# CSB5/XNA_Basecaller

Hardware: AMD Instinct MI355X
Metric: raw signal samples/sec basecalled, chunksize 10k (higher is better)
Workload: dtype f32 (feed-forward projections split-f16x3 MFMA, recurrent projections f16 MFMA + FP8 block-scaled correction MFMA, f32 accumulate; CRF decode f32)

## Files before the change

### xna_basecaller_amd/csrc/xb_encoder.hip

```cpp
#include "xb_enc_common.h"

namespace {

constexpr int CF_TT = 32;

__global__ __launch_bounds__(256) void conv_front_kernel(xb::ConvFrontParams p)
{
    extern __shared__ __attribute__((aligned(16))) unsigned char smem_raw[];
    const int tid = threadIdx.x;
    const int n = blockIdx.y;
    const int t0 = blockIdx.x * CF_TT;
    const int W = p.winlen, ST = p.stride, pad = W / 2, L = p.L;
    const int nq = (CF_TT - 1) * ST + W;
    const int q0 = t0 * ST - pad;
    float *sig = reinterpret_cast<float *>(smem_raw);
    float *a1 = sig + nq + 8;
    float *a2 = a1 + 4 * (nq + 4);
    float *w2s = a2 + 16 * nq;
    float *b2s = w2s + 320, *w1s = b2s + 16, *b1s = w1s + 20;

    for (int i = tid; i < 320; i += 256) w2s[i] = p.w2[i];
    if (tid < 16) b2s[tid] = p.b2[tid];
    if (tid < 20) w1s[tid] = p.w1[tid];
    if (tid < 4) b1s[tid] = p.b1[tid];
    const float *x = (p.signal2 && n >= p.split) ? p.signal2 + (size_t)(n - p.split) * L : p.signal + (size_t)n * L;
    for (int i = tid; i < nq + 8; i += 256) {
        const int pos = q0 - 4 + i;
        sig[i] = (pos >= 0 && pos < L) ? x[pos] : 0.0f;
    }
    __syncthreads();
    for (int i = tid; i < 4 * (nq + 4); i += 256) {
        const int c = i / (nq + 4), r = i % (nq + 4);
        const int pos = q0 - 2 + r;
        float v = 0.0f;
        if (pos >= 0 && pos < L) {
            float acc = b1s[c];
#pragma unroll
            for (int k = 0; k < 5; ++k) acc += w1s[c * 5 + k] * sig[r + k];
            v = silu(acc);
        }
        a1[c * (nq + 4) + r] = v;
    }
    __syncthreads();
    for (int i = tid; i < 16 * nq; i += 256) {
        const int c = i / nq, r = i % nq;
        const int pos = q0 + r;
        float v = 0.0f;
        if (pos >= 0 && pos < L) {
            float acc = b2s[c];
#pragma unroll
            for (int ci = 0; ci < 4; ++ci)
#pragma unroll
                for (int k = 0; k < 5; ++k) acc += w2s[(c * 4 + ci) * 5 + k] * a1[ci * (nq + 4) + r + k];
            v = silu(acc);
        }
        a2[c * nq + r] = v;
    }
    __syncthreads();
    const int kp = p.kp, kv = 16 * W, kq = kp / 4;
    for (int i = tid; i < CF_TT * kq; i += 256) {
        const int tt = i / kq, col = (i % kq) * 4;
        const int t = t0 + tt;
        if (t >= p.T) break;
        float v[4];
#pragma unroll
        for (int j = 0; j < 4; ++j) {
            const int cj = col + j;
            v[j] = cj < kv ? a2[(cj / W) * nq + tt * ST + cj % W] : 0.0f;
        }
        const size_t orow = (size_t)t * p.N + n;
        half_t hi[4];
        unsigned short hb[4];
        if (p.q8) {
            float lo[4];
#pragma unroll
            for (int j = 0; j < 4; ++j) {
                hi[j] = (half_t)v[j];
                lo[j] = clamp448((v[j] - (float)hi[j]) * 2048.0f);
                hb[j] = __builtin_bit_cast(unsigned short, hi[j]);
            }
            unsigned h8 = fp8_pair<false>(clamp448((float)hi[0]), clamp448((float)hi[1]), 0u);
            h8 = fp8_pair<true>(clamp448((float)hi[2]), clamp448((float)hi[3]), h8);
            unsigned l8 = fp8_pair<false>(lo[0], lo[1], 0u);
            l8 = fp8_pair<true>(lo[2], lo[3], l8);
            unsigned char *q = reinterpret_cast<unsigned char *>(p.a_lo) + q8_offset(orow, kp, col);
            *reinterpret_cast<unsigned *>(q) = h8;
            *reinterpret_cast<unsigned *>(q + 32) = l8;
        } else {
            unsigned short lb[4];
#pragma unroll
            for (int j = 0; j < 4; ++j) {
                half_t lo;
                split_f16(v[j], hi[j], lo);
                hb[j] = __builtin_bit_cast(unsigned short, hi[j]);
                lb[j] = __builtin_bit_cast(unsigned short, lo);
            }
            *reinterpret_cast<uint2 *>(p.a_lo + orow * kp + col) =
                make_uint2(lb[0] | ((unsigned)lb[1] << 16), lb[2] | ((unsigned)lb[3] << 16));
        }
        *reinterpret_cast<uint2 *>(p.a_hi + orow * kp + col) =
            make_uint2(hb[0] | ((unsigned)hb[1] << 16), hb[2] | ((unsigned)hb[3] << 16));
    }
}

constexpr int GBM = 256, GBN = 256, GBK = 32, GTHREADS = 512;


__host__ __device__ inline int gemm_super_n(int NT) { return NT % 2 == 0 ? 2 : (NT % 3 == 0 ? 3 : 1); }

__device__ __forceinline__ bool gemm_tile_origin(const xb::GemmParams &p, int &m0, int &n0)
{
    const int MT = (p.M + GBM - 1) / GBM, NT = (p.Nn + GBN - 1) / GBN;
    const int SN = gemm_super_n(NT), SM = 32 / SN;
    const int ngroups = (NT + SN - 1) / SN, msup = (MT + SM - 1) / SM;
    const int b = blockIdx.x, xcd = b & 7, j = b >> 3;
    const int q = (j >> 5) * 8 + xcd, w = j & 31;
    if (q >= msup * ngroups || w >= SM * SN) return false;
    const int mt = (q / ngroups) * SM + w / SN, nt = (q % ngroups) * SN + w % SN;
    if (mt >= MT || nt >= NT) return false;
    m0 = mt * GBM;
    n0 = nt * GBN;
    return true;
}

template <bool L16>
__device__ __forceinline__ constexpr int acc_row(int r) { return L16 ? (r & 7) + 16 * (r >> 3) : (r & 3) + 8 * (r >> 2); }

__device__ __forceinline__ void acc16_lines(const f32x4 (&a)[8][4], floatx16 (&o)[4][2])
{
    asm volatile("s_nop 7\n\ts_nop 7");
#pragma unroll
    for (int i = 0; i < 4; ++i)
#pragma unroll
        for (int jp = 0; jp < 2; ++jp)
#pragma unroll
            for (int ib = 0; ib < 2; ++ib)
#pragma unroll
                for (int r = 0; r < 4; ++r) {
                    float u = a[2 * i + ib][2 * jp][r], v = a[2 * i + ib][2 * jp + 1][r];
                    asm volatile("v_permlane16_swap_b32 %0, %1" : "+v"(u), "+v"(v));
                    o[i][jp][ib * 8 + r] = u;
                    o[i][jp][ib * 8 + 4 + r] = v;
                }
}

template <int EPI, bool L16 = false>
__device__ __forceinline__ void gemm_epilogue(const xb::GemmParams &p, const floatx16 (&acc)[4][2], int mw, int nw, int lane)
{
    constexpr int HS = L16 ? 8 : 4;
    if (mw >= p.M || nw >= p.Nn) return;
    float bj[2];
#pragma unroll
    for (int j = 0; j < 2; ++j) {
        const int n = nw + j * 32 + (lane & 31);
        bj[j] = (p.bias && n < p.Nn) ? p.bias[n] : 0.0f;
    }
    const bool interior = mw + 128 <= p.M && nw + 64 <= p.Nn;
    const bool out_q8 = p.out_fmt ? p.out_fmt == 2 : p.nsplit == 2;
    if (EPI == xb::EPI_BIAS_F32 && interior && (p.gin_n == 0 || p.gin_n >= 43)) {
        const int ld = p.gin_n ? 128 : p.ldc;
        float *tile;
        int c0 = 0, n = 1 << 30;
        long long wrap = 0;
        if (p.gin_n) {
            n = p.gin_n;
            const int t0 = mw / n;
            c0 = mw - t0 * n;
            const int MB = p.Nn >> 7;
            tile = p.out_f32 + (((size_t)t0 * MB + (size_t)(nw >> 7)) * n + c0) * 128 + (nw & 127);
            wrap = (long long)(MB - 1) * n * 128;
        } else {
            tile = p.out_f32 + (size_t)mw * p.ldc + nw;
        }
        const int loff = (HS * (lane >> 5)) * ld + (lane & 31);
        if (c0 + 128 <= n) {
#pragma unroll
            for (int i = 0; i < 4; ++i)
#pragma unroll
                for (int r = 0; r < 16; ++r) {
                    float *rowp = tile + (size_t)(i * 32 + acc_row<L16>(r)) * ld;
#pragma unroll
                    for (int j = 0; j < 2; ++j) __builtin_nontemporal_store(acc[i][j][r] + bj[j], rowp + loff + j * 32);
                }
        } else {
            const int cl = c0 + HS * (lane >> 5);
#pragma unroll
            for (int i = 0; i < 4; ++i)
#pragma unroll
                for (int r = 0; r < 16; ++r) {
                    const int rr = i * 32 + acc_row<L16>(r);
                    const int c = cl + rr;
                    const int k = (c >= n) + (c >= 2 * n) + (c >= 3 * n);
                    float *rowp = tile + (size_t)rr * ld + (long long)k * wrap;
#pragma unroll
                    for (int j = 0; j < 2; ++j) __builtin_nontemporal_store(acc[i][j][r] + bj[j], rowp + loff + j * 32);
                }
        }
        return;
    }
    if (EPI == xb::EPI_TANH_SCALE && interior && !p.expand) {
        float *tile = p.out_f32 + (size_t)mw * p.ldc + nw;
        const int loff = (HS * (lane >> 5)) * p.ldc + (lane & 31);
#pragma unroll
        for (int i = 0; i < 4; ++i)
#pragma unroll
            for (int r = 0; r < 16; ++r) {
                float *rowp = tile + (size_t)(i * 32 + acc_row<L16>(r)) * p.ldc;
#pragma unroll
                for (int j = 0; j < 2; ++j) rowp[loff + j * 32] = p.scale * fast_tanh(acc[i][j][r] + bj[j]);
            }
        return;
    }
    if (EPI == xb::EPI_SILU_SPLIT && interior) {
        const size_t tile = (size_t)mw * p.ldc + nw;
        const int loff = (HS * (lane >> 5)) * p.ldc + (lane & 31);
        unsigned char *q8base = reinterpret_cast<unsigned char *>(p.out_lo) + tile * 2;
        const int qoff = (HS * (lane >> 5)) * p.ldc * 2 + (lane & 31);
#pragma unroll
        for (int i = 0; i < 4; ++i)
#pragma unroll
            for (int r = 0; r < 16; ++r) {
                const size_t ro = (size_t)(i * 32 + acc_row<L16>(r)) * p.ldc;
#pragma unroll
                for (int j = 0; j < 2; ++j) {
                    const float v = silu(acc[i][j][r] + bj[j]);
                    if (out_q8) {
                        half_t hi;
                        unsigned char h8, l8;
                        q8_bytes(v, p.out_exp, hi, h8, l8);
                        p.out_hi[tile + ro + loff + j * 32] = hi;
                        unsigned char *q = q8base + ro * 2 + qoff + j * 64;
                        q[0] = h8;
                        q[32] = l8;
                    } else {
                        half_t hi, lo;
                        split_f16(v, hi, lo);
                        p.out_hi[tile + ro + loff + j * 32] = hi;
                        p.out_lo[tile + ro + loff + j * 32] = lo;
                    }
                }
            }
        return;
    }
#pragma unroll
    for (int i = 0; i < 4; ++i)
#pragma unroll
        for (int j = 0; j < 2; ++j) {
            const int n = nw + j * 32 + (lane & 31);
            if (n >= p.Nn) continue;
            const float bias = bj[j];
            int ocol = n;
            if (EPI == xb::EPI_TANH_SCALE && p.expand) ocol = (n / p.nb) * (p.nb + 1) + 1 + n % p.nb;
#pragma unroll
            for (int r = 0; r < 16; ++r) {
                const int m = mw + i * 32 + acc_row<L16>(r) + HS * (lane >> 5);
                if (m >= p.M) continue;
                const float v = acc[i][j][r] + bias;
                if (EPI == xb::EPI_BIAS_F32) {
                    p.out_f32[p.gin_n ? xb::gin_offset((size_t)m, n, p.gin_n, p.Nn) : (size_t)m * p.ldc + n] = v;
                } else if (EPI == xb::EPI_SILU_SPLIT) {
                    if (out_q8) {
                        half_t hi;
                        unsigned char h8, l8;
                        q8_bytes(silu(v), p.out_exp, hi, h8, l8);
                        unsigned char *q = reinterpret_cast<unsigned char *>(p.out_lo) + q8_offset((size_t)m, p.ldc, n);
                        p.out_hi[(size_t)m * p.ldc + n] = hi;
                        q[0] = h8;
                        q[32] = l8;
                    } else {
                        half_t hi, lo;
                        split_f16(silu(v), hi, lo);
                        p.out_hi[(size_t)m * p.ldc + n] = hi;
                        p.out_lo[(size_t)m * p.ldc + n] = lo;
                    }
                } else {
                    p.out_f32[(size_t)m * p.ldc + ocol] = p.scale * fast_tanh(v);
                    if (p.expand && n % p.nb == 0) p.out_f32[(size_t)m * p.ldc + ocol - 1] = p.blank;
                }
            }
        }
}

#define G8_BARRIER()                                   \
    do {                                               \
        __builtin_amdgcn_sched_barrier(0);             \
        __builtin_amdgcn_s_barrier();                  \
        __builtin_amdgcn_sched_barrier(0);             \
    } while (0)

template <int EPI, int NSPLIT>
__global__ __launch_bounds__(GTHREADS) void gemm8r_kernel(xb::GemmParams p)
{
    constexpr int NP = NSPLIT == 1 ? 1 : 2;
    constexpr int PARTB = 128 * 64;
    constexpr int HTB = NP * PARTB;
    extern __shared__ __attribute__((aligned(16))) unsigned char smem_raw[];
    const int tid = threadIdx.x, lane = tid & 63;
    const int wid = __builtin_amdgcn_readfirstlane(tid >> 6);
    const int wr = wid >> 2, wc = wid & 3;
    int m0, n0;
    if (!gemm_tile_origin(p, m0, n0)) return;
    const int nk = p.K / GBK;

    unsigned offs[4];
    {
        const int drow = 16 * wid + (lane >> 2), dch = ((lane & 3) ^ ((lane >> 4) & 3)) * 8;
        const int Mrem = p.M - 1 - m0, Nrem = p.Nn - 1 - n0;
        int r;
        r = drow;        offs[0] = (unsigned)(((r > Mrem ? Mrem : r) * p.lda + dch) * 2);
        r = 128 + drow;  offs[1] = (unsigned)(((r > Mrem ? Mrem : r) * p.lda + dch) * 2);
        r = drow;        offs[2] = (unsigned)(((r > Nrem ? Nrem : r) * p.ldb + dch) * 2);
        r = 128 + drow;  offs[3] = (unsigned)(((r > Nrem ? Nrem : r) * p.ldb + dch) * 2);
    }
    const unsigned char *const tA_hi = reinterpret_cast<const unsigned char *>(p.a_hi + (size_t)m0 * p.lda);
    const unsigned char *const tA_lo = reinterpret_cast<const unsigned char *>(p.a_lo + (size_t)m0 * p.lda);
    const unsigned char *const tB_hi = reinterpret_cast<const unsigned char *>(p.b_hi + (size_t)n0 * p.ldb);
    const unsigned char *const tB_lo = reinterpret_cast<const unsigned char *>(p.b_lo + (size_t)n0 * p.ldb);
    unsigned char *const wdst = smem_raw + wid * 1024;
    u32x4 st[4][NP];
    unsigned char *const ldst = wdst + lane * 16;
#define G8_LOAD(h, t)                                                                           \
    do {                                                                                        \
        const size_t kb_ = (size_t)(t) * (GBK * 2);                                             \
        st[(h)][0] = *reinterpret_cast<const u32x4 *>(((h) < 2 ? tA_hi : tB_hi) + kb_ + offs[(h)]); \
        if (NP == 2) st[(h)][1] = *reinterpret_cast<const u32x4 *>(((h) < 2 ? tA_lo : tB_lo) + kb_ + offs[(h)]); \
    } while (0)
#define G8_WRITE(h, t)                                                                          \
    do {                                                                                        \
        unsigned char *dst_ = ldst + (((h) * 2 + ((t) & 1)) * HTB);                             \
        *reinterpret_cast<u32x4 *>(dst_) = st[(h)][0];                                          \
        if (NP == 2) *reinterpret_cast<u32x4 *>(dst_ + PARTB) = st[(h)][1];                     \
    } while (0)

    unsigned la[2];
#pragma unroll
    for (int ks = 0; ks < 2; ++ks)
        la[ks] = (unsigned)((lane & 31) * 64 + (((2 * ks + (lane >> 5)) ^ ((lane >> 2) & 3)) * 16));
    constexpr bool S16 = NSPLIT == 3;
    const unsigned la16 = (unsigned)((lane & 15) * 64 + (((lane >> 4) ^ ((lane >> 2) & 3)) * 16));
    const unsigned char *const fragA = smem_raw + wr * 2 * HTB;
    const unsigned char *const fragB = smem_raw + (2 + (wc >> 1)) * 2 * HTB + (wc & 1) * 4096;

    unsigned lqa[2], lqb[2];
#pragma unroll
    for (int j = 0; j < 2; ++j) {
        const int h = lane >> 5, sw = (lane >> 2) & 3;
        lqa[j] = (unsigned)((lane & 31) * 64 + (((2 * h + j) ^ sw) * 16));
        lqb[j] = (unsigned)((lane & 31) * 64 + (((2 * (1 - h) + j) ^ sw) * 16));
    }
    const int sca = 127 - p.a_exp - 11, scb = 127 - p.b_exp;

    half8 ah[2][2], al[2][2], bh[2], bl[2];
    v8i aq[2], bq;
#define G8_READ_A(d, mh)                                                                                  \
    _Pragma("unroll") for (int i2 = 0; i2 < 2; ++i2) {                                                    \
        const unsigned char *t_ = fragA + (d) * HTB + ((mh) * 2 + i2) * 2048;                         \
        _Pragma("unroll") for (int ks = 0; ks < 2; ++ks) {                                                \
            ah[i2][ks] = *reinterpret_cast<const half8 *>(t_ + (S16 ? ks * 1024 + la16 : la[ks]));        \
            if (S16) al[i2][ks] = *reinterpret_cast<const half8 *>(t_ + PARTB + ks * 1024 + la16);       \
        }                                                                                                 \
        if (NSPLIT == 2) {                                                                                \
            const v4i x_ = *reinterpret_cast<const v4i *>(t_ + PARTB + lqa[0]);                           \
            const v4i y_ = *reinterpret_cast<const v4i *>(t_ + PARTB + lqa[1]);                           \
            aq[i2] = __builtin_shufflevector(x_, y_, 0, 1, 2, 3, 4, 5, 6, 7);                             \
        }                                                                                                 \
    }
#define G8_READ_B(d, n)                                                                                   \
    do {                                                                                                  \
        const unsigned char *t_ = fragB + (d) * HTB + (n) * 2048;                                     \
        _Pragma("unroll") for (int ks = 0; ks < 2; ++ks) {                                                \
            bh[ks] = *reinterpret_cast<const half8 *>(t_ + (S16 ? ks * 1024 + la16 : la[ks]));            \
            if (S16) bl[ks] = *reinterpret_cast<const half8 *>(t_ + PARTB + ks * 1024 + la16);           \
        }                                                                                                 \
        if (NSPLIT == 2) {                                                                                \
            const v4i x_ = *reinterpret_cast<const v4i *>(t_ + PARTB + lqb[0]);                           \
            const v4i y_ = *reinterpret_cast<const v4i *>(t_ + PARTB + lqb[1]);                           \
            bq = __builtin_shufflevector(x_, y_, 0, 1, 2, 3, 4, 5, 6, 7);                            \
        }                                                                                                 \
    } while (0)
#define G8_F16(i2, ks, n, A_, B_)                                                                         \
    acc[(mh_) * 2 + (i2)][(n)] = __builtin_amdgcn_mfma_f32_32x32x16_f16(A_[(i2)][(ks)], B_[(ks)], acc[(mh_) * 2 + (i2)][(n)], 0, 0, 0)
#define G8_S16(A_, B_, n)                                                                                 \
    _Pragma("unroll") for (int i4 = 0; i4 < 4; ++i4)                                                      \
        _Pragma("unroll") for (int j2 = 0; j2 < 2; ++j2)                                                  \
            acc16[mh_ * 4 + i4][(n) * 2 + j2] = __builtin_amdgcn_mfma_f32_16x16x32_f16(A_[i4 >> 1][i4 & 1], B_[j2], acc16[mh_ * 4 + i4][(n) * 2 + j2], 0, 0, 0)
#define G8_MFMA(mh, n)                                                                                    \
    do {                                                                                                  \
        constexpr int mh_ = (mh);                                                                         \
        __builtin_amdgcn_s_setprio(1);                                                                    \
        if constexpr (S16) {                                                                              \
            G8_S16(al, bh, n);                                                                            \
            G8_S16(ah, bl, n);                                                                            \
            G8_S16(ah, bh, n);                                                                            \
        } else if (NSPLIT == 2) {                                                                                \
            G8_F16(0, 0, n, ah, bh);                                                                      \
            G8_F16(1, 0, n, ah, bh);                                                                      \
            _Pragma("unroll") for (int i2 = 0; i2 < 2; ++i2) acc[mh_ * 2 + i2][(n)] =                     \
                __builtin_amdgcn_mfma_scale_f32_32x32x64_f8f6f4(aq[i2], bq, acc[mh_ * 2 + i2][(n)], 0, 0, 0, sca, 0, scb); \
            G8_F16(0, 1, n, ah, bh);                                                                      \
            G8_F16(1, 1, n, ah, bh);                                                                      \
        } else {                                                                                          \
            _Pragma("unroll") for (int ks = 0; ks < 2; ++ks) {                                            \
                G8_F16(0, ks, n, ah, bh);                                                                 \
                G8_F16(1, ks, n, ah, bh);                                                                 \
            }                                                                                             \
        }                                                                                                 \
        __builtin_amdgcn_s_setprio(0);                                                                    \
    } while (0)

    floatx16 acc[4][2];
    f32x4 acc16[8][4];
#pragma unroll
    for (int i = 0; i < 4; ++i)
#pragma unroll
        for (int j = 0; j < 2; ++j)
#pragma unroll
            for (int r = 0; r < 16; ++r) acc[i][j][r] = 0.0f;
#pragma unroll
    for (int i = 0; i < 8; ++i)
#pragma unroll
        for (int j = 0; j < 4; ++j)
#pragma unroll
            for (int r = 0; r < 4; ++r) acc16[i][j][r] = 0.0f;

#pragma unroll
    for (int h = 0; h < 4; ++h) G8_LOAD(h, 0);
#pragma unroll
    for (int h = 0; h < 4; ++h) G8_WRITE(h, 0);
#pragma unroll
    for (int h = 0; h < 4; ++h) G8_LOAD(h, nk > 1 ? 1 : 0);
    asm volatile("s_waitcnt lgkmcnt(0)" ::: "memory");
    G8_BARRIER();
    if (wr == 1) G8_BARRIER();
// ... 193 lines not shown
    _Pragma("unroll") for (int i_ = 0; i_ < 2; ++i_)                                            \
        _Pragma("unroll") for (int j_ = 0; j_ < 2; ++j_)                                        \
            _Pragma("unroll") for (int c_ = 0; c_ < 2; ++c_)                                    \
                acc16[(q) * 2 + i_][2 * j_ + c_] = __builtin_amdgcn_mfma_f32_16x16x32_f16(      \
                    A_[i_], __builtin_bit_cast(half8, bS[j_][(pc0) + c_]), acc16[(q) * 2 + i_][2 * j_ + c_], 0, 0, 0)
#define G4P_S16(AH_, AL_, q, bS)                                                                \
    do {                                                                                        \
        G4P_M16(AL_, q, bS, 0);                                                                 \
        G4P_M16(AH_, q, bS, 2);                                                                 \
        G4P_M16(AH_, q, bS, 0);                                                                 \
    } while (0)
#define G4P_WAIT8(n, bS)                                                                        \
    asm volatile("s_waitcnt vmcnt(%8)" : "+v"(bS[0][0]), "+v"(bS[1][0]), "+v"(bS[0][1]), "+v"(bS[1][1]), \
                 "+v"(bS[0][2]), "+v"(bS[1][2]), "+v"(bS[0][3]), "+v"(bS[1][3]) : "i"(n))
#define G4P_MFMA_BEGIN() do { G4P_SB(); __builtin_amdgcn_s_setprio(1); } while (0)
#define G4P_MFMA_END() do { __builtin_amdgcn_s_setprio(0); G4P_SB(); } while (0)

#define G4P_TILE(bS, t)                                                                         \
    do {                                                                                        \
        const unsigned char *const sa = smem_raw + cur * STB;                                   \
        const int t2_ = (t) + 2 < nk ? (t) + 2 : nk - 1;                                        \
        const unsigned char *const b2 = tB + (size_t)t2_ * bks;                                 \
         \
        const bool live_ = (t) + 2 < nk;                                                        \
        const unsigned vb_ = live_ ? voff0 : 0u;                                                \
        if ((t) == 0) G4P_STAMP(0);                                                             \
        if constexpr (!S16) {                                                                   \
            asm volatile("s_waitcnt vmcnt(%0)" ::"i"(2 * NB + NA) : "memory");                  \
            G4P_SB();                                                                           \
            __builtin_amdgcn_s_barrier();                                                       \
            G4P_SB();                                                                           \
            G4P_STAMP(1);                                                                       \
        }                                                                                       \
        if constexpr (NSPLIT == 2) {                                                            \
            dma_a(t2_, nxt2, live_);           \
             \
             \
            half8 h0[2], h1[2], g0[2], g1[2];                                                   \
            v8i q0[2], q1[2];                                                                   \
            G4P_RD_H(h0, sa, 0, 0, 0);                                                          \
            G4P_RD_H(h1, sa, 0, 1, 0);                                                          \
            G4P_WAIT2(INFL - 2, bS[0][0], bS[1][0]);                                            \
            G4P_MFMA_BEGIN();                                                                   \
            G4P_F16(h0, 0, bS, 0);                                                              \
            G4P_MFMA_END();                                                                     \
            G4P_RD_Q(q0, sa, 0);                                                                \
            G4P_RD_Q(q1, sa, 1);                                                                \
            G4P_MFMA_BEGIN();                                                                   \
            G4P_F16(h1, 1, bS, 0);                                                              \
            G4P_MFMA_END();                                                                     \
            G4P_LDB_GROUP_V(bS, vb_, b2, 0);                                                           \
            G4P_WAIT4(INFL - 4, bS[0][2], bS[0][3], bS[1][2], bS[1][3]);                        \
            G4P_MFMA_BEGIN();                                                                   \
            G4P_F8(q0, 0, bS);                                                                  \
            G4P_MFMA_END();                                                                     \
            G4P_RD_H(g0, sa, 0, 0, 1);                                                          \
            G4P_RD_H(g1, sa, 0, 1, 1);                                                          \
            G4P_MFMA_BEGIN();                                                                   \
            G4P_F8(q1, 1, bS);                                                                  \
            G4P_MFMA_END();                                                                     \
            G4P_LDB_GROUP_V(bS, vb_, b2, 2);                                                           \
            G4P_LDB_GROUP_V(bS, vb_, b2, 3);                                                           \
            G4P_WAIT2(INFL - 2, bS[0][1], bS[1][1]);                                            \
            G4P_MFMA_BEGIN();                                                                   \
            G4P_F16(g0, 0, bS, 1);                                                              \
            G4P_F16(g1, 1, bS, 1);                                                              \
            G4P_MFMA_END();                                                                     \
            G4P_LDB_GROUP_V(bS, vb_, b2, 1);                                                           \
        } else if constexpr (S16) {                                                             \
             \
             \
             \
             \
             \
             \
             \
             \
            half8 yh[2], yl[2];                                                                 \
            G4P_RD16(yl, sa, 1, 1);                                                             \
            G4P_RD16(yh, sa, 0, 1);                                                             \
            G4P_WAIT8(INFL - 8 - NA, bS);                                                       \
            G4P_STAMP(2);                                                                       \
            G4P_MFMA_BEGIN();                                                                   \
            G4P_S16(xh, xl, 0, bS);                                                             \
            G4P_MFMA_END();                                                                     \
            dma_a(t2_, nxt2, live_);                                                            \
            G4P_RD16(xl, sa, 1, 2);                                                             \
            G4P_RD16(xh, sa, 0, 2);                                                             \
            G4P_MFMA_BEGIN();                                                                   \
            G4P_S16(yh, yl, 1, bS);                                                             \
            G4P_MFMA_END();                                                                     \
            G4P_RD16(yl, sa, 1, 3);                                                             \
            G4P_RD16(yh, sa, 0, 3);                                                             \
            G4P_MFMA_BEGIN();                                                                   \
            G4P_S16(xh, xl, 2, bS);                                                             \
            G4P_MFMA_END();                                                                     \
            G4P_STAMP(3);                                                                       \
            asm volatile("s_waitcnt vmcnt(%0)\n\ts_waitcnt lgkmcnt(0)" ::"i"(NB + NA) : "memory"); \
            G4P_SB();                                                                           \
            __builtin_amdgcn_s_barrier();                                                       \
            G4P_SB();                                                                           \
            G4P_STAMP(1);                                                                       \
            const unsigned char *const sn = smem_raw + nxt1 * STB;                              \
            G4P_RD16(xl, sn, 1, 0);                                                             \
            G4P_RD16(xh, sn, 0, 0);                                                             \
            G4P_MFMA_BEGIN();                                                                   \
            G4P_M16(yl, 3, bS, 0);                                                              \
            G4P_M16(yh, 3, bS, 2);                                                              \
            G4P_MFMA_END();                                                                     \
            G4P_LDB_GROUP_V(bS, vb_, b2, 2);                                                    \
            G4P_LDB_GROUP_V(bS, vb_, b2, 3);                                                    \
            G4P_MFMA_BEGIN();                                                                   \
            G4P_M16(yh, 3, bS, 0);                                                              \
            G4P_MFMA_END();                                                                     \
            G4P_LDB_GROUP_V(bS, vb_, b2, 0);                                                    \
            G4P_LDB_GROUP_V(bS, vb_, b2, 1);                                                    \
        } else {                                                                                \
             \
             \
             \
             \
            half8 ah0[2], ah1[2];                                                               \
            G4P_RD_H(ah0, sa, 0, 0, 0);                                                         \
            G4P_RD_H(ah1, sa, 0, 1, 0);                                                         \
            _Pragma("unroll") for (int ks = 0; ks < 2; ++ks) {                                  \
                 \
                 \
                constexpr int LA_ = NA;                                                         \
                if (ks == 0) G4P_WAIT2(INFL - 2 - LA_, bS[0][0], bS[1][0]);                     \
                else G4P_WAIT2(INFL - 2, bS[0][1], bS[1][1]);                                   \
                G4P_MFMA_BEGIN();                                                               \
                G4P_F16(ah0, 0, bS, ks);                                                        \
                G4P_MFMA_END();                                                                 \
                if (ks == 0) {                                                                  \
                    dma_a(t2_, nxt2, live_);                                                    \
                    G4P_RD_H(ah0, sa, 0, 0, 1);                                                 \
                }                                                                               \
                G4P_MFMA_BEGIN();                                                               \
                G4P_F16(ah1, 1, bS, ks);                                                        \
                G4P_MFMA_END();                                                                 \
                if (ks == 0) {                                                                  \
                    G4P_RD_H(ah1, sa, 0, 1, 1);                                                 \
                    G4P_LDB_GROUP_V(bS, vb_, b2, 0);                                            \
                } else {                                                                        \
                    G4P_LDB_GROUP_V(bS, vb_, b2, 1);                                            \
                }                                                                               \
            }                                                                                   \
        }                                                                                       \
        if constexpr (!S16) asm volatile("s_waitcnt lgkmcnt(0)" ::: "memory");                  \
        G4P_STAMP(3);                                                                           \
        { const int c_ = cur; cur = nxt1; nxt1 = nxt2; nxt2 = c_; }                             \
    } while (0)

    if (__builtin_amdgcn_readfirstlane(n0 + wid * 64 >= p.Nn ? 1 : 0)) {
        dma_a(0, 0);
        dma_a(nk > 1 ? 1 : 0, 1);
        int c0 = 0, c1 = 1, c2 = 2;
#pragma unroll 1
        for (int t = 0; t < nk + (S16 ? 1 : 0); ++t) {
            asm volatile("s_waitcnt vmcnt(%0)" ::"i"(NA) : "memory");
            __builtin_amdgcn_s_barrier();
            dma_a(t + 2 < nk ? t + 2 : nk - 1, c2, t + 2 < nk);
            const int c_ = c0; c0 = c1; c1 = c2; c2 = c_;
        }
        asm volatile("s_waitcnt vmcnt(0)" ::: "memory");
        return;
    }

    int cur = 0, nxt1 = 1, nxt2 = 2;
    {
        const int t1 = nk > 1 ? 1 : 0;
        const unsigned char *const b0 = tB, *const b1 = tB + (size_t)t1 * bks;
        dma_a(0, 0);
        if constexpr (NSPLIT == 2) {
            G4P_LDB_GROUP(bE, b0, 0); G4P_LDB_GROUP(bE, b0, 2); G4P_LDB_GROUP(bE, b0, 3); G4P_LDB_GROUP(bE, b0, 1);
        } else if constexpr (S16) {
            G4P_LDB_GROUP(bE, b0, 2); G4P_LDB_GROUP(bE, b0, 3); G4P_LDB_GROUP(bE, b0, 0); G4P_LDB_GROUP(bE, b0, 1);
        } else {
            G4P_LDB_GROUP(bE, b0, 0); G4P_LDB_GROUP(bE, b0, 1);
        }
        dma_a(t1, 1);
        if constexpr (NSPLIT == 2) {
            G4P_LDB_GROUP(bO, b1, 0); G4P_LDB_GROUP(bO, b1, 2); G4P_LDB_GROUP(bO, b1, 3); G4P_LDB_GROUP(bO, b1, 1);
        } else if constexpr (S16) {
            G4P_LDB_GROUP(bO, b1, 2); G4P_LDB_GROUP(bO, b1, 3); G4P_LDB_GROUP(bO, b1, 0); G4P_LDB_GROUP(bO, b1, 1);
        } else {
            G4P_LDB_GROUP(bO, b1, 0); G4P_LDB_GROUP(bO, b1, 1);
        }
    }
    if constexpr (S16) {
        asm volatile("s_waitcnt vmcnt(%0)" ::"i"(2 * NB + NA) : "memory");
        G4P_SB();
        __builtin_amdgcn_s_barrier();
        G4P_SB();
        G4P_RD16(xl, smem_raw, 1, 0);
        G4P_RD16(xh, smem_raw, 0, 0);
    }
    int t = 0;
#pragma unroll 1
    for (; t + 1 < nk; t += 2) {
        G4P_TILE(bE, t);
        G4P_TILE(bO, t + 1);
    }
    if (t < nk) G4P_TILE(bE, t);
    if constexpr (NSPLIT == 1)
        asm volatile("s_waitcnt vmcnt(0)" : "+v"(bE[0][0]), "+v"(bE[1][0]), "+v"(bE[0][1]), "+v"(bE[1][1]),
                       "+v"(bO[0][0]), "+v"(bO[1][0]), "+v"(bO[0][1]), "+v"(bO[1][1]) :: "memory");
    else
        asm volatile("s_waitcnt vmcnt(0)" : "+v"(bE[0][0]), "+v"(bE[1][0]), "+v"(bE[0][1]), "+v"(bE[1][1]),
                       "+v"(bE[0][2]), "+v"(bE[1][2]), "+v"(bE[0][3]), "+v"(bE[1][3]),
                       "+v"(bO[0][0]), "+v"(bO[1][0]), "+v"(bO[0][1]), "+v"(bO[1][1]),
                       "+v"(bO[0][2]), "+v"(bO[1][2]), "+v"(bO[0][3]), "+v"(bO[1][3]) :: "memory");
    G4P_SB();
#undef G4P_TILE
#undef G4P_LDB
#undef G4P_LDB_GROUP
#undef G4P_LDB_GROUP_V
#undef G4P_WAIT2
#undef G4P_WAIT4
#undef G4P_RD_H
#undef G4P_RD16
#undef G4P_M16
#undef G4P_S16
#undef G4P_WAIT8
#undef G4P_RD_Q
#undef G4P_F16
#undef G4P_F8
#undef G4P_MFMA_BEGIN
#undef G4P_MFMA_END
#undef G4P_SB

    int lane_e = lane, mw_e = m0, nw_e = n0 + wid * 64;
    asm volatile("" : "+v"(lane_e), "+s"(mw_e), "+s"(nw_e));
    if constexpr (S16) acc16_lines(acc16, acc);
    gemm_epilogue<EPI, S16>(p, acc, mw_e, nw_e, lane_e);
#ifdef XB_GEMM_STAMPS
    if (NSPLIT == 3) {
        asm volatile("s_waitcnt vmcnt(0)" ::: "memory");
        G4P_STAMP(4);
        if (tid == 0) {
            for (int i = 0; i < 5; ++i) atomicAdd(&g_gemm_stamps[i], st_acc[i]);
            atomicAdd(&g_gemm_stamps[5], (unsigned long long)(__builtin_amdgcn_s_getreg(4 | (0 << 6) | (3 << 11)) & 1u));
            atomicAdd(&g_gemm_stamps[6], 1ull);
            atomicAdd(&g_gemm_stamps[7], (unsigned long long)nk);
        }
    }
#endif
}

template <int EPI, int NSPLIT>
hipError_t launch_gemm_ns(const xb::GemmParams &p, hipStream_t stream)
{
    const int MT = (p.M + GBM - 1) / GBM, NT = (p.Nn + GBN - 1) / GBN;
    const int SN = gemm_super_n(NT), SM = 32 / SN;
    const int supers = ((NT + SN - 1) / SN) * ((MT + SM - 1) / SM);
    dim3 grid(8 * 32 * ((supers + 7) / 8)), block(GTHREADS);
    const size_t lds = (size_t)2 * 4 * (NSPLIT == 1 ? 1 : 2) * 128 * 64;
    (void)hipFuncSetAttribute(reinterpret_cast<const void *>(&gemm8r_kernel<EPI, NSPLIT>),
                              hipFuncAttributeMaxDynamicSharedMemorySize, (int)lds);
    hipLaunchKernelGGL((gemm8r_kernel<EPI, NSPLIT>), grid, block, lds, stream, p);
    return hipGetLastError();
}

template <int EPI, int NSPLIT>
hipError_t launch_gemm4p_ns(const xb::GemmParams &p, hipStream_t stream)
{
    const int MT = (p.M + G4_BM - 1) / G4_BM, NT = (p.Nn + G4_BN - 1) / G4_BN;
    const int snw = p.sn > 0 ? p.sn : gemm_super_n(NT);
    const int SN = NT < snw ? NT : snw, SM = 64 / SN;
    const int supers = ((NT + SN - 1) / SN) * ((MT + SM - 1) / SM);
    dim3 grid(8 * 64 * ((supers + 7) / 8)), block(G4_THREADS);
    size_t lds = (size_t)3 * (NSPLIT == 1 ? 1 : 2) * 128 * 64;
    if (p.one_per_cu) {
        lds = 96 * 1024;
        (void)hipFuncSetAttribute(reinterpret_cast<const void *>(&gemm4p_kernel<EPI, NSPLIT>),
                                  hipFuncAttributeMaxDynamicSharedMemorySize, (int)lds);
    }
    hipLaunchKernelGGL((gemm4p_kernel<EPI, NSPLIT>), grid, block, lds, stream, p);
    return hipGetLastError();
}

template <int EPI>
hipError_t launch_gemm_epi(const xb::GemmParams &p, hipStream_t stream)
{
    if (p.b4) {
        switch (p.nsplit) {
        case 1: return launch_gemm4p_ns<EPI, 1>(p, stream);
        case 2: return launch_gemm4p_ns<EPI, 2>(p, stream);
        default: return launch_gemm4p_ns<EPI, 3>(p, stream);
        }
    }
    switch (p.nsplit) {
    case 1: return launch_gemm_ns<EPI, 1>(p, stream);
    case 2: return launch_gemm_ns<EPI, 2>(p, stream);
    default: return launch_gemm_ns<EPI, 3>(p, stream);
    }
}

}


namespace xb {

#ifdef XB_GEMM_STAMPS
void gemm_read_stamps(unsigned long long out[8], bool reset)
{
    hipMemcpyFromSymbol(out, HIP_SYMBOL(g_gemm_stamps), sizeof(unsigned long long) * 8);
    if (reset) {
        unsigned long long z[8] = {};
        hipMemcpyToSymbol(HIP_SYMBOL(g_gemm_stamps), z, sizeof z);
    }
}
#endif

hipError_t launch_conv_front(const ConvFrontParams &p, hipStream_t stream)
{
    if (p.N < 1 || p.T < 1 || p.kp < 16 * p.winlen || p.kp % 32 != 0) return hipErrorInvalidValue;
    const int nq = (CF_TT - 1) * p.stride + p.winlen;
    const size_t lds = sizeof(float) * ((size_t)(nq + 8) + 4 * (nq + 4) + 16 * (size_t)nq + 360);
    if (lds > 60000) return hipErrorInvalidValue;
    dim3 grid((p.T + CF_TT - 1) / CF_TT, p.N), block(256);
    hipLaunchKernelGGL(conv_front_kernel, grid, block, lds, stream, p);
    return hipGetLastError();
}

hipError_t launch_gemm(const GemmParams &p, int epilogue, hipStream_t stream)
{
    if (p.M < 1 || p.Nn < 1 || p.K < GBK || p.K % GBK != 0 || p.lda % 8 != 0 || p.ldb % 8 != 0 ||
        p.lda < p.K || p.ldb < p.K)
        return hipErrorInvalidValue;
    if (p.nsplit < 1 || p.nsplit > 3) return hipErrorInvalidValue;
    switch (epilogue) {
    case EPI_BIAS_F32: return launch_gemm_epi<EPI_BIAS_F32>(p, stream);
    case EPI_SILU_SPLIT: return launch_gemm_epi<EPI_SILU_SPLIT>(p, stream);
    case EPI_TANH_SCALE: return launch_gemm_epi<EPI_TANH_SCALE>(p, stream);
    default: return hipErrorInvalidValue;
    }
}

}
```

Baseline: 43.28 million.

## Overlap GEMM epilogue stores with final k-tile MFMAs in split-f16 path

Refactors the GEMM epilogue into a struct with per-row-block store methods. The S16 kernel path peels the last k-tile and interleaves its MFMA groups with accumulator permutation and stores for completed row blocks, so epilogue global writes overlap the tail compute. It also reorders the B prefetch for odd tile counts and removes redundant DMA and extra barrier iterations in the idle-wave path. This adds register pressure and complexity in the tail and risks hazards around the permlane swaps on accumulators that are still being written.

Result: no change. 43.68 million, median of 6 (+0.9%).

```diff
diff --git a/xna_basecaller_amd/csrc/xb_encoder.hip b/xna_basecaller_amd/csrc/xb_encoder.hip
--- a/xna_basecaller_amd/csrc/xb_encoder.hip
+++ b/xna_basecaller_amd/csrc/xb_encoder.hip
@@ -126,66 +126,97 @@
 template <bool L16>
 __device__ __forceinline__ constexpr int acc_row(int r) { return L16 ? (r & 7) + 16 * (r >> 3) : (r & 3) + 8 * (r >> 2); }
 
+__device__ __forceinline__ void acc16_block(const f32x4 (&a)[8][4], floatx16 (&o)[2], int i)
+{
+    asm volatile("s_nop 7\n\ts_nop 7\n\ts_nop 7");
+#pragma unroll
+    for (int jp = 0; jp < 2; ++jp)
+#pragma unroll
+        for (int ib = 0; ib < 2; ++ib)
+#pragma unroll
+            for (int r = 0; r < 4; ++r) {
+                float u = a[2 * i + ib][2 * jp][r], v = a[2 * i + ib][2 * jp + 1][r];
+                asm volatile("v_permlane16_swap_b32 %0, %1" : "+v"(u), "+v"(v));
+                o[jp][ib * 8 + r] = u;
+                o[jp][ib * 8 + 4 + r] = v;
+            }
+}
+
 __device__ __forceinline__ void acc16_lines(const f32x4 (&a)[8][4], floatx16 (&o)[4][2])
 {
-    asm volatile("s_nop 7\n\ts_nop 7");
-#pragma unroll
-    for (int i = 0; i < 4; ++i)
-#pragma unroll
-        for (int jp = 0; jp < 2; ++jp)
-#pragma unroll
-            for (int ib = 0; ib < 2; ++ib)
-#pragma unroll
-                for (int r = 0; r < 4; ++r) {
-                    float u = a[2 * i + ib][2 * jp][r], v = a[2 * i + ib][2 * jp + 1][r];
-                    asm volatile("v_permlane16_swap_b32 %0, %1" : "+v"(u), "+v"(v));
-                    o[i][jp][ib * 8 + r] = u;
-                    o[i][jp][ib * 8 + 4 + r] = v;
-                }
+#pragma unroll
+    for (int i = 0; i < 4; ++i) acc16_block(a, o[i], i);
 }
 
 template <int EPI, bool L16 = false>
-__device__ __forceinline__ void gemm_epilogue(const xb::GemmParams &p, const floatx16 (&acc)[4][2], int mw, int nw, int lane)
-{
-    constexpr int HS = L16 ? 8 : 4;
-    if (mw >= p.M || nw >= p.Nn) return;
+struct GemmEpilogue {
+    static constexpr int HS = L16 ? 8 : 4;
     float bj[2];
-#pragma unroll
-    for (int j = 0; j < 2; ++j) {
-        const int n = nw + j * 32 + (lane & 31);
-        bj[j] = (p.bias && n < p.Nn) ? p.bias[n] : 0.0f;
-    }
-    const bool interior = mw + 128 <= p.M && nw + 64 <= p.Nn;
-    const bool out_q8 = p.out_fmt ? p.out_fmt == 2 : p.nsplit == 2;
-    if (EPI == xb::EPI_BIAS_F32 && interior && (p.gin_n == 0 || p.gin_n >= 43)) {
-        const int ld = p.gin_n ? 128 : p.ldc;
-        float *tile;
-        int c0 = 0, n = 1 << 30;
-        long long wrap = 0;
-        if (p.gin_n) {
-            n = p.gin_n;
-            const int t0 = mw / n;
-            c0 = mw - t0 * n;
-            const int MB = p.Nn >> 7;
-            tile = p.out_f32 + (((size_t)t0 * MB + (size_t)(nw >> 7)) * n + c0) * 128 + (nw & 127);
-            wrap = (long long)(MB - 1) * n * 128;
-        } else {
-            tile = p.out_f32 + (size_t)mw * p.ldc + nw;
-        }
-        const int loff = (HS * (lane >> 5)) * ld + (lane & 31);
-        if (c0 + 128 <= n) {
-#pragma unroll
-            for (int i = 0; i < 4; ++i)
+    bool live, fast, interior, out_q8, gin_rows;
+    int mw, nw, lane;
+    float *tile;
+    int ld, c0, n;
+    long long wrap;
+    size_t base;
+    int loff;
+
+    __device__ __forceinline__ void load_bias(const xb::GemmParams &p, int nw_, int lane_)
+    {
+#pragma unroll
+        for (int j = 0; j < 2; ++j) {
+            const int col = nw_ + j * 32 + (lane_ & 31);
+            bj[j] = p.bias ? p.bias[col < p.Nn ? col : p.Nn - 1] : 0.0f;
+        }
+    }
+
+    __device__ __forceinline__ void init(const xb::GemmParams &p, int mw_, int nw_, int lane_)
+    {
+        mw = mw_, nw = nw_, lane = lane_;
+        live = !(mw >= p.M || nw >= p.Nn);
+        fast = false;
+        if (!live) return;
+        interior = mw + 128 <= p.M && nw + 64 <= p.Nn;
+        out_q8 = p.out_fmt ? p.out_fmt == 2 : p.nsplit == 2;
+        gin_rows = EPI == xb::EPI_BIAS_F32 && interior && (p.gin_n == 0 || p.gin_n >= 43);
+        fast = gin_rows || (EPI == xb::EPI_TANH_SCALE && interior && !p.expand) || (EPI == xb::EPI_SILU_SPLIT && interior);
+        base = (size_t)mw * p.ldc + nw;
+        loff = (HS * (lane >> 5)) * p.ldc + (lane & 31);
+        if (gin_rows) {
+            ld = p.gin_n ? 128 : p.ldc;
+            c0 = 0, n = 1 << 30;
+            wrap = 0;
+            if (p.gin_n) {
+                n = p.gin_n;
+                const int t0 = mw / n;
+                c0 = mw - t0 * n;
+                const int MB = p.Nn >> 7;
+                tile = p.out_f32 + (((size_t)t0 * MB + (size_t)(nw >> 7)) * n + c0) * 128 + (nw & 127);
+                wrap = (long long)(MB - 1) * n * 128;
+            } else {
+                tile = p.out_f32 + base;
+            }
+            loff = (HS * (lane >> 5)) * ld + (lane & 31);
+        }
+    }
+
+    __device__ __forceinline__ void rows(const xb::GemmParams &p, const floatx16 (&acc)[2], int i) const
+    {
+        if (fast) rows_interior(p, acc, i);
+        else rows_edge(p, acc, i);
+    }
+
+    __device__ __forceinline__ void rows_interior(const xb::GemmParams &p, const floatx16 (&acc)[2], int i) const
+    {
+        if (EPI == xb::EPI_BIAS_F32 && gin_rows) {
+            if (c0 + 128 <= n) {
 #pragma unroll
                 for (int r = 0; r < 16; ++r) {
                     float *rowp = tile + (size_t)(i * 32 + acc_row<L16>(r)) * ld;
 #pragma unroll
-                    for (int j = 0; j < 2; ++j) __builtin_nontemporal_store(acc[i][j][r] + bj[j], rowp + loff + j * 32);
+                    for (int j = 0; j < 2; ++j) __builtin_nontemporal_store(acc[j][r] + bj[j], rowp + loff + j * 32);
                 }
-        } else {
-            const int cl = c0 + HS * (lane >> 5);
-#pragma unroll
-            for (int i = 0; i < 4; ++i)
+            } else {
+                const int cl = c0 + HS * (lane >> 5);
 #pragma unroll
                 for (int r = 0; r < 16; ++r) {
                     const int rr = i * 32 + acc_row<L16>(r);
@@ -193,92 +224,99 @@
                     const int k = (c >= n) + (c >= 2 * n) + (c >= 3 * n);
                     float *rowp = tile + (size_t)rr * ld + (long long)k * wrap;
 #pragma unroll
-                    for (int j = 0; j < 2; ++j) __builtin_nontemporal_store(acc[i][j][r] + bj[j], rowp + loff + j * 32);
+                    for (int j = 0; j < 2; ++j) __builtin_nontemporal_store(acc[j][r] + bj[j], rowp + loff + j * 32);
                 }
-        }
-        return;
-    }
-    if (EPI == xb::EPI_TANH_SCALE && interior && !p.expand) {
-        float *tile = p.out_f32 + (size_t)mw * p.ldc + nw;
-        const int loff = (HS * (lane >> 5)) * p.ldc + (lane & 31);
-#pragma unroll
-        for (int i = 0; i < 4; ++i)
+            }
+            return;
+        }
+        if (EPI == xb::EPI_TANH_SCALE && interior && !p.expand) {
+            float *t_ = p.out_f32 + base;
 #pragma unroll
             for (int r = 0; r < 16; ++r) {
-                float *rowp = tile + (size_t)(i * 32 + acc_row<L16>(r)) * p.ldc;
-#pragma unroll
-                for (int j = 0; j < 2; ++j) rowp[loff + j * 32] = p.scale * fast_tanh(acc[i][j][r] + bj[j]);
+                float *rowp = t_ + (size_t)(i * 32 + acc_row<L16>(r)) * p.ldc;
+#pragma unroll
+                for (int j = 0; j < 2; ++j) rowp[loff + j * 32] = p.scale * fast_tanh(acc[j][r] + bj[j]);
             }
-        return;
-    }
-    if (EPI == xb::EPI_SILU_SPLIT && interior) {
-        const size_t tile = (size_t)mw * p.ldc + nw;
-        const int loff = (HS * (lane >> 5)) * p.ldc + (lane & 31);
-        unsigned char *q8base = reinterpret_cast<unsigned char *>(p.out_lo) + tile * 2;
-        const int qoff = (HS * (lane >> 5)) * p.ldc * 2 + (lane & 31);
-#pragma unroll
-        for (int i = 0; i < 4; ++i)
+            return;
+        }
+        if (EPI == xb::EPI_SILU_SPLIT && interior) {
+            unsigned char *q8base = reinterpret_cast<unsigned char *>(p.out_lo) + base * 2;
+            const int qoff = (HS * (lane >> 5)) * p.ldc * 2 + (lane & 31);
 #pragma unroll
             for (int r = 0; r < 16; ++r) {
                 const size_t ro = (size_t)(i * 32 + acc_row<L16>(r)) * p.ldc;
 #pragma unroll
                 for (int j = 0; j < 2; ++j) {
-                    const float v = silu(acc[i][j][r] + bj[j]);
+                    const float v = silu(acc[j][r] + bj[j]);
                     if (out_q8) {
                         half_t hi;
                         unsigned char h8, l8;
                         q8_bytes(v, p.out_exp, hi, h8, l8);
-                        p.out_hi[tile + ro + loff + j * 32] = hi;
+                        p.out_hi[base + ro + loff + j * 32] = hi;
                         unsigned char *q = q8base + ro * 2 + qoff + j * 64;
                         q[0] = h8;
                         q[32] = l8;
                     } else {
                         half_t hi, lo;
                         split_f16(v, hi, lo);
-                        p.out_hi[tile + ro + loff + j * 32] = hi;
-                        p.out_lo[tile + ro + loff + j * 32] = lo;
+                        p.out_hi[base + ro + loff + j * 32] = hi;
+                        p.out_lo[base + ro + loff + j * 32] = lo;
                     }
                 }
             }
-        return;
-    }
-#pragma unroll
-    for (int i = 0; i < 4; ++i)
+            return;
+        }
+    }
+
+    __device__ __forceinline__ void rows_edge(const xb::GemmParams &p, const floatx16 (&acc)[2], int i) const
+    {
+        if (!live) return;
 #pragma unroll
         for (int j = 0; j < 2; ++j) {
-            const int n = nw + j * 32 + (lane & 31);
-            if (n >= p.Nn) continue;
+            const int col = nw + j * 32 + (lane & 31);
+            if (col >= p.Nn) continue;
             const float bias = bj[j];
-            int ocol = n;
-            if (EPI == xb::EPI_TANH_SCALE && p.expand) ocol = (n / p.nb) * (p.nb + 1) + 1 + n % p.nb;
+            int ocol = col;
+            if (EPI == xb::EPI_TANH_SCALE && p.expand) ocol = (col / p.nb) * (p.nb + 1) + 1 + col % p.nb;
 #pragma unroll
             for (int r = 0; r < 16; ++r) {
                 const int m = mw + i * 32 + acc_row<L16>(r) + HS * (lane >> 5);
                 if (m >= p.M) continue;
-                const float v = acc[i][j][r] + bias;
+                const float v = acc[j][r] + bias;
                 if (EPI == xb::EPI_BIAS_F32) {
-                    p.out_f32[p.gin_n ? xb::gin_offset((size_t)m, n, p.gin_n, p.Nn) : (size_t)m * p.ldc + n] = v;
+                    p.out_f32[p.gin_n ? xb::gin_offset((size_t)m, col, p.gin_n, p.Nn) : (size_t)m * p.ldc + col] = v;
                 } else if (EPI == xb::EPI_SILU_SPLIT) {
                     if (out_q8) {
                         half_t hi;
                         unsigned char h8, l8;
                         q8_bytes(silu(v), p.out_exp, hi, h8, l8);
-                        unsigned char *q = reinterpret_cast<unsigned char *>(p.out_lo) + q8_offset((size_t)m, p.ldc, n);
-                        p.out_hi[(size_t)m * p.ldc + n] = hi;
+                        unsigned char *q = reinterpret_cast<unsigned char *>(p.out_lo) + q8_offset((size_t)m, p.ldc, col);
+                        p.out_hi[(size_t)m * p.ldc + col] = hi;
                         q[0] = h8;
                         q[32] = l8;
                     } else {
                         half_t hi, lo;
                         split_f16(silu(v), hi, lo);
-                        p.out_hi[(size_t)m * p.ldc + n] = hi;
-                        p.out_lo[(size_t)m * p.ldc + n] = lo;
+                        p.out_hi[(size_t)m * p.ldc + col] = hi;
+                        p.out_lo[(size_t)m * p.ldc + col] = lo;
                     }
                 } else {
                     p.out_f32[(size_t)m * p.ldc + ocol] = p.scale * fast_tanh(v);
-                    if (p.expand && n % p.nb == 0) p.out_f32[(size_t)m * p.ldc + ocol - 1] = p.blank;
+                    if (p.expand && col % p.nb == 0) p.out_f32[(size_t)m * p.ldc + ocol - 1] = p.blank;
                 }
             }
         }
+    }
+};
+
+template <int EPI, bool L16 = false>
+__device__ __forceinline__ void gemm_epilogue(const xb::GemmParams &p, const floatx16 (&acc)[4][2], int mw, int nw, int lane)
+{
+    GemmEpilogue<EPI, L16> e;
+    e.load_bias(p, nw, lane);
+    e.init(p, mw, nw, lane);
+#pragma unroll
+    for (int i = 0; i < 4; ++i) e.rows(p, acc[i], i);
 }
 
 #define G8_BARRIER()                                   \
@@ -778,25 +816,85 @@
         { const int c_ = cur; cur = nxt1; nxt1 = nxt2; nxt2 = c_; }                             \
     } while (0)
 
+#define G4P_DRAIN()                                                                             \
+    asm volatile("s_waitcnt vmcnt(0)" : "+v"(bE[0][0]), "+v"(bE[1][0]), "+v"(bE[0][1]), "+v"(bE[1][1]), \
+                   "+v"(bE[0][2]), "+v"(bE[1][2]), "+v"(bE[0][3]), "+v"(bE[1][3]),              \
+                   "+v"(bO[0][0]), "+v"(bO[1][0]), "+v"(bO[0][1]), "+v"(bO[1][1]),              \
+                   "+v"(bO[0][2]), "+v"(bO[1][2]), "+v"(bO[0][3]), "+v"(bO[1][3]) :: "memory")
+#define G4P_STORE(q)                                                                            \
+    do {                                                                                        \
+        acc16_block(acc16, o_[(q)], (q));                                                       \
+        if (epi.fast) epi.rows_interior(p, o_[(q)], (q));                                       \
+    } while (0)
+#define G4P_LAST(bS, t)                                                                         \
+    do {                                                                                        \
+        const unsigned char *const sa = smem_raw + cur * STB;                                   \
+        if ((t) == 0) G4P_STAMP(0);                                                             \
+        half8 yh[2], yl[2];                                                                     \
+        G4P_RD16(yl, sa, 1, 1);                                                                 \
+        G4P_RD16(yh, sa, 0, 1);                                                                 \
+        G4P_WAIT8(INFL - 8 - NA, bS);                                                           \
+        G4P_STAMP(2);                                                                           \
+         \
+         \
+        int lane_e = lane, mw_e = m0, nw_e = n0 + wid * 64;                                     \
+        asm volatile("" : "+v"(lane_e), "+s"(mw_e), "+s"(nw_e));                                \
+        GemmEpilogue<EPI, true> epi;                                                            \
+        epi.load_bias(p, nw_e, lane_e);                                                         \
+        G4P_MFMA_BEGIN();                                                                       \
+        G4P_S16(xh, xl, 0, bS);                                                                 \
+        G4P_MFMA_END();                                                                         \
+        G4P_RD16(xl, sa, 1, 2);                                                                 \
+        G4P_RD16(xh, sa, 0, 2);                                                                 \
+        epi.init(p, mw_e, nw_e, lane_e);                                                        \
+        G4P_DRAIN();                                                                            \
+        asm volatile("" : "+v"(epi.bj[0]), "+v"(epi.bj[1]));                                    \
+         \
+         \
+        floatx16 o_[4][2];                                                                      \
+        G4P_MFMA_BEGIN();                                                                       \
+        G4P_S16(yh, yl, 1, bS);                                                                 \
+        G4P_MFMA_END();                                                                         \
+        G4P_RD16(yl, sa, 1, 3);                                                                 \
+        G4P_RD16(yh, sa, 0, 3);                                                                 \
+        G4P_STORE(0);                                                                           \
+        G4P_MFMA_BEGIN();                                                                       \
+        G4P_S16(xh, xl, 2, bS);                                                                 \
+        G4P_MFMA_END();                                                                         \
+        G4P_STORE(1);                                                                           \
+        G4P_MFMA_BEGIN();                                                                       \
+        G4P_M16(yl, 3, bS, 0);                                                                  \
+        G4P_M16(yh, 3, bS, 2);                                                                  \
+        G4P_M16(yh, 3, bS, 0);                                                                  \
+        G4P_MFMA_END();                                                                         \
+        G4P_STAMP(3);                                                                           \
+        G4P_STORE(2);                                                                           \
+        G4P_STORE(3);                                                                           \
+        if (!epi.fast) {                                                                        \
+            _Pragma("unroll") for (int q_ = 0; q_ < 4; ++q_) epi.rows_edge(p, o_[q_], q_);      \
+        }                                                                                       \
+    } while (0)
+
     if (__builtin_amdgcn_readfirstlane(n0 + wid * 64 >= p.Nn ? 1 : 0)) {
         dma_a(0, 0);
-        dma_a(nk > 1 ? 1 : 0, 1);
+        if (nk > 1) dma_a(1, 1);
         int c0 = 0, c1 = 1, c2 = 2;
 #pragma unroll 1
-        for (int t = 0; t < nk + (S16 ? 1 : 0); ++t) {
-            asm volatile("s_waitcnt vmcnt(%0)" ::"i"(NA) : "memory");
+        for (int t = 0; t < nk; ++t) {
+            if (t + 1 < nk) asm volatile("s_waitcnt vmcnt(%0)" ::"i"(NA) : "memory");
+            else asm volatile("s_waitcnt vmcnt(0)" ::: "memory");
             __builtin_amdgcn_s_barrier();
-            dma_a(t + 2 < nk ? t + 2 : nk - 1, c2, t + 2 < nk);
+            if (t + 2 < nk) dma_a(t + 2, c2);
             const int c_ = c0; c0 = c1; c1 = c2; c2 = c_;
         }
-        asm volatile("s_waitcnt vmcnt(0)" ::: "memory");
         return;
     }
 
     int cur = 0, nxt1 = 1, nxt2 = 2;
+    const bool odd = S16 && (nk & 1);
     {
         const int t1 = nk > 1 ? 1 : 0;
-        const unsigned char *const b0 = tB, *const b1 = tB + (size_t)t1 * bks;
+        const unsigned char *const b0 = tB + (size_t)(odd ? t1 : 0) * bks, *const b1 = tB + (size_t)(odd ? 0 : t1) * bks;
         dma_a(0, 0);
         if constexpr (NSPLIT == 2) {
             G4P_LDB_GROUP(bE, b0, 0); G4P_LDB_GROUP(bE, b0, 2); G4P_LDB_GROUP(bE, b0, 3); G4P_LDB_GROUP(bE, b0, 1);
@@ -823,22 +921,45 @@
         G4P_RD16(xh, smem_raw, 0, 0);
     }
     int t = 0;
+    if constexpr (S16) {
+        if (odd) {
+            G4P_DRAIN();
+            if (nk > 1) {
+                G4P_TILE(bO, t);
+                t = 1;
+            }
+        }
 #pragma unroll 1
-    for (; t + 1 < nk; t += 2) {
-        G4P_TILE(bE, t);
-        G4P_TILE(bO, t + 1);
-    }
-    if (t < nk) G4P_TILE(bE, t);
-    if constexpr (NSPLIT == 1)
-        asm volatile("s_waitcnt vmcnt(0)" : "+v"(bE[0][0]), "+v"(bE[1][0]), "+v"(bE[0][1]), "+v"(bE[1][1]),
-                       "+v"(bO[0][0]), "+v"(bO[1][0]), "+v"(bO[0][1]), "+v"(bO[1][1]) :: "memory");
-    else
-        asm volatile("s_waitcnt vmcnt(0)" : "+v"(bE[0][0]), "+v"(bE[1][0]), "+v"(bE[0][1]), "+v"(bE[1][1]),
-                       "+v"(bE[0][2]), "+v"(bE[1][2]), "+v"(bE[0][3]), "+v"(bE[1][3]),
-                       "+v"(bO[0][0]), "+v"(bO[1][0]), "+v"(bO[0][1]), "+v"(bO[1][1]),
-                       "+v"(bO[0][2]), "+v"(bO[1][2]), "+v"(bO[0][3]), "+v"(bO[1][3]) :: "memory");
+        for (; t + 2 < nk; t += 2) {
+            G4P_TILE(bE, t);
+            G4P_TILE(bO, t + 1);
+        }
+        if (t + 1 < nk) {
+            G4P_TILE(bE, t);
+            ++t;
+        }
+        G4P_LAST(bO, t);
+    } else {
+#pragma unroll 1
+        for (; t + 1 < nk; t += 2) {
+            G4P_TILE(bE, t);
+            G4P_TILE(bO, t + 1);
+        }
+        if (t < nk) G4P_TILE(bE, t);
+        if constexpr (NSPLIT == 1)
+            asm volatile("s_waitcnt vmcnt(0)" : "+v"(bE[0][0]), "+v"(bE[1][0]), "+v"(bE[0][1]), "+v"(bE[1][1]),
+                           "+v"(bO[0][0]), "+v"(bO[1][0]), "+v"(bO[0][1]), "+v"(bO[1][1]) :: "memory");
+        else
+            asm volatile("s_waitcnt vmcnt(0)" : "+v"(bE[0][0]), "+v"(bE[1][0]), "+v"(bE[0][1]), "+v"(bE[1][1]),
+                           "+v"(bE[0][2]), "+v"(bE[1][2]), "+v"(bE[0][3]), "+v"(bE[1][3]),
+                           "+v"(bO[0][0]), "+v"(bO[1][0]), "+v"(bO[0][1]), "+v"(bO[1][1]),
+                           "+v"(bO[0][2]), "+v"(bO[1][2]), "+v"(bO[0][3]), "+v"(bO[1][3]) :: "memory");
+    }
     G4P_SB();
 #undef G4P_TILE
+#undef G4P_LAST
+#undef G4P_STORE
+#undef G4P_DRAIN
 #undef G4P_LDB
 #undef G4P_LDB_GROUP
 #undef G4P_LDB_GROUP_V
@@ -856,10 +977,11 @@
 #undef G4P_MFMA_END
 #undef G4P_SB
 
-    int lane_e = lane, mw_e = m0, nw_e = n0 + wid * 64;
-    asm volatile("" : "+v"(lane_e), "+s"(mw_e), "+s"(nw_e));
-    if constexpr (S16) acc16_lines(acc16, acc);
-    gemm_epilogue<EPI, S16>(p, acc, mw_e, nw_e, lane_e);
+    if constexpr (!S16) {
+        int lane_e = lane, mw_e = m0, nw_e = n0 + wid * 64;
+        asm volatile("" : "+v"(lane_e), "+s"(mw_e), "+s"(nw_e));
+        gemm_epilogue<EPI, false>(p, acc, mw_e, nw_e, lane_e);
+    }
 #ifdef XB_GEMM_STAMPS
     if (NSPLIT == 3) {
         asm volatile("s_waitcnt vmcnt(0)" ::: "memory");
```
